# CC834/Heterogeneous-OpenCL-Image-Processing-Engine

Measured on AMD Instinct MI355X. Metric: images_per_sec, higher is better.
Workload: dtype u8

## Files before the change

### heterogeneous-opencl-image-processing-engine_amd/__init__.py

```python
from __future__ import annotations

import ctypes as C
import os
import re
import subprocess

PKG_DIR = os.path.dirname(os.path.abspath(__file__))
ROOT = os.path.dirname(PKG_DIR)
CSRC = os.path.join(PKG_DIR, "csrc")
APPS = os.path.join(PKG_DIR, "apps")
LIB_PATH = os.path.join(PKG_DIR, "libmi_blur.so")
HEADER = os.path.join(ROOT, "include", "mi_blur.h")
HIPCC = os.environ.get("HIPCC", "/opt/rocm/bin/hipcc")
os.environ.setdefault("HIP_FORCE_DEV_KERNARG", "0")
ARCH = "gfx950"

DEVICE_CPU = -1
VARIANT_AUTO, VARIANT_GENERIC, VARIANT_TILED, VARIANT_STREAM, VARIANT_DIRECT = 0, 1, 2, 3, 4
OK, ERR_INVALID, ERR_NO_DEVICE, ERR_NOMEM, ERR_STATE, ERR_UNSUPPORTED = 0, -1, -2, -3, -4, -5
UNIQUE_ID_BYTES = 128
SEP_MAX_RADIUS = 16
MEDIAN_MAX_RADIUS = 7
MORPH_MAX_RADIUS = 16
MORPH_ERODE, MORPH_DILATE, MORPH_GRADIENT = 0, 1, 2
# ... 319 lines not shown
        "mi_blur_warp_perspective_quad": (i, [C.POINTER(C.c_double), C.POINTER(C.c_double), C.POINTER(C.c_double)]),
        "mi_blur_warp_perspective_set_matrix": (i, [C.POINTER(WarpPerspective), C.POINTER(C.c_double), i]),
        "mi_blur_enqueue_warp_perspective": (i, [u8p, u8p, i, i, i, i, C.POINTER(WarpPerspective), vp]),
        "mi_blur_cpu_run_warp_perspective": (i, [u8p, u8p, i, i, i, i, C.POINTER(WarpPerspective), i]),
        "mi_blur_ctx_set_warp_perspective": (i, [vp, C.POINTER(WarpPerspective)]),
        "mi_blur_conv_preset": (i, [i, C.POINTER(Conv)]),
        "mi_blur_enqueue_conv": (i, [u8p, u8p, i, i, i, i, C.POINTER(Conv), vp]),
        "mi_blur_enqueue_conv_band": (i, [u8p, u8p, i, i, i, i, i, C.POINTER(Conv), vp]),
        "mi_blur_cpu_run_conv": (i, [u8p, u8p, i, i, i, i, C.POINTER(Conv), i]),
        "mi_blur_ctx_set_conv": (i, [vp, C.POINTER(Conv)]),
        "mi_blur_fill_synthetic": (None, [u8p, i, i, i, i, i, i]),
        "mi_blur_fnv1a64": (C.c_uint64, [u8p, C.c_size_t]),
        "mi_blur_debug_zc_trace": (i, [vp, C.POINTER(C.c_uint64), i, C.POINTER(i), C.POINTER(C.c_uint)]),
        "mi_blur_debug_xcd_times": (i, [C.POINTER(C.c_uint64), C.POINTER(C.c_uint64), i]),
        "mi_blur_debug_xcd_raw": (i, [C.POINTER(C.c_uint64), C.c_size_t, C.c_size_t]),
        "mi_blur_a1_partition": (None, [i, i, C.c_float, C.POINTER(i), C.POINTER(i)]),
        "mi_blur_shard_range": (None, [C.c_longlong, i, i, C.POINTER(C.c_longlong), C.POINTER(C.c_longlong)]),
        "mi_blur_a2_split": (None, [i, C.c_float, i, C.POINTER(A2Geometry)]),
        "mi_blur_band_of": (None, [i, i, i, i, C.POINTER(Band)]),
        "mi_blur_comm_unique_id": (i, [vp]),
        "mi_blur_comm_init_rank": (i, [C.POINTER(vp), i, i, vp]),
        "mi_blur_comm_init_all": (i, [C.POINTER(vp), i, C.POINTER(i)]),
        "mi_blur_comm_init_p2p": (i, [C.POINTER(vp), i, C.POINTER(i)]),
        "mi_blur_comm_init_pull": (i, [C.POINTER(vp), i, C.POINTER(i)]),
        "mi_blur_comm_destroy": (None, [vp]),
        "mi_blur_comm_info": (i, [vp, C.POINTER(i), C.POINTER(i), C.POINTER(i)]),
        "mi_blur_halo_exchange": (i, [vp, u8p, i, i, i, i, vp]),
        "mi_blur_peer_export": (i, [vp, vp, C.POINTER(C.c_uint64)]),
        "mi_blur_peer_open": (i, [vp, C.c_uint64, C.POINTER(vp)]),
        "mi_blur_peer_close": (i, [vp, C.c_uint64]),
# ... 471 lines not shown
```

### heterogeneous-opencl-image-processing-engine_amd/csrc/blur_kernels.hip

```cpp
#include "kernel_common.h"

#include <math.h>
#include <stdlib.h>
#include <string.h>
#include <mutex>
#include <algorithm>

namespace mi_blur {

__device__ __forceinline__ u16x2 as_pk(uint32_t x) { return __builtin_bit_cast(u16x2, x); }
__device__ __forceinline__ uint32_t as_u32(u16x2 x) { return __builtin_bit_cast(uint32_t, x); }

constexpr uint32_t EVEN_MASK = 0x00ff00ffu;
__device__ __forceinline__ uint32_t even_of(uint32_t x) { return x & EVEN_MASK; }
__device__ __forceinline__ uint32_t odd_of(uint32_t x) { return __builtin_amdgcn_perm(0u, x, 0x0c030c01u); }
__device__ __forceinline__ uint32_t mad6(uint32_t c, uint32_t t) { return as_u32(as_pk(c) * (unsigned short)6 + as_pk(t)); }

constexpr uint32_t sel_left(int C, int q)
{
    uint32_t s = 0;
    for (int j = 0; j < 4; j++) {
        int p = -4 * q + j;
        int idx = ((p % C) + C) % C;
        s |= (uint32_t)idx << (8 * j);
// ... 309 lines not shown
        }
    }
}

constexpr unsigned XCD_DEBUG_SLOTS = 1u << 20;
__device__ __forceinline__ void xcd_time_mark(unsigned long long *t, unsigned long long t0)
{
    if (threadIdx.x == 0 && blockIdx.x < XCD_DEBUG_SLOTS) {
        unsigned id;
        asm volatile("s_getreg_b32 %0, hwreg(HW_REG_XCC_ID)" : "=s"(id));
        t[2u * blockIdx.x] = ((unsigned long long)__builtin_amdgcn_s_memrealtime() << 4) | (id & 7u);
        t[2u * blockIdx.x + 1] = t0;
    }
}

template <int C, int R, int RPG, bool DMA, bool SHFL = false, bool RAG = false>
__global__ __launch_bounds__(256) void blur_tiled_kernel(const TiledParams p)
{
    const unsigned long long t0 = p.xcd_times ? __builtin_amdgcn_s_memrealtime() : 0ull;
    tiled_tile<C, R, RPG, DMA, SHFL, RAG>(p, xcd_map(blockIdx.x, p.nblocks, p.xcd));
    if (p.xcd_times) xcd_time_mark(p.xcd_times, t0);
}

template <int C, int R, int RPG>
__global__ __launch_bounds__(256) void blur_tiled_loop_kernel(const TiledParams p)
{
    for (unsigned L = blockIdx.x; L < p.nblocks; L += gridDim.x) {
        tiled_tile<C, R, RPG, true, false, false>(p, L);
        __syncthreads();
    }
}

template <int C, int R, int RPG, int X>
__global__ __launch_bounds__(256) void blur_tiled_x_kernel(const TiledParams p)
// ... 434 lines not shown
    }
    wait_vmcnt<0>();
}

struct DirectParams {
    const uint8_t *in;
    uint8_t *out;
    long long in_stride, out_stride;
    long long total;
    int pitch, cpr;
    int H, y0, y1;
    int nbands;
    unsigned nblocks;
    int xcd;
    const uint8_t *top, *bottom;
};

template <int C, int R, int BH, bool PEER = false>
__global__ __launch_bounds__(256) void blur_direct_kernel(const DirectParams p)
{
    constexpr int WIN = 2 * R + 1, NR = BH + 2 * R;
    const int lane = threadIdx.x & 63, wave = threadIdx.x >> 6;
    const unsigned B = xcd_map(blockIdx.x, p.nblocks, p.xcd);
    const long long fl = (long long)(B * 4u + (unsigned)wave) * 62 - 1 + lane;
    const bool inrange = fl >= 0 && fl < p.total;
    const unsigned f = (unsigned)(fl < 0 ? 0 : (fl >= p.total ? p.total - 1 : fl));
    const unsigned col = f % (unsigned)p.cpr, t2 = f / (unsigned)p.cpr;
    const unsigned band = t2 % (unsigned)p.nbands;
    const long long img = (long long)(t2 / (unsigned)p.nbands);
    const bool compute = inrange && lane >= 1 && lane <= 62;
    const int row0 = p.y0 + (int)band * BH;
    const int rows_out = compute ? min(BH, p.y1 - row0) : 0;
    const bool at_start = col == 0, at_end = (int)col == p.cpr - 1;
    const bool any_edge = __builtin_amdgcn_ballot_w64(at_start || at_end) != 0ull;
    const uint8_t *src = p.in + img * p.in_stride + (size_t)col * 16u;
    uint8_t *dst = p.out + img * p.out_stride + (size_t)(row0 - p.y0) * (size_t)p.pitch + (size_t)col * 16u;
// ... 36 lines not shown
                    const uint32_t se = (((hw[(j + 2) % WIN][q] << 1) + hw[(j + 1) % WIN][q]) + hw[j % WIN][q]) << 4;
                    const uint32_t so = (((hw[(j + 2) % WIN][4 + q] << 1) + hw[(j + 1) % WIN][4 + q]) + hw[j % WIN][4 + q]) << 4;
                    o[q] = __builtin_amdgcn_perm(so, se, 0x07030501u);
                } else {
                    const uint32_t se = mad6(hw[(j + 3) % WIN][q], ((hw[(j + 2) % WIN][q] + hw[(j + 4) % WIN][q]) << 2) + (hw[(j + 1) % WIN][q] + hw[j % WIN][q]));
                    const uint32_t so = mad6(hw[(j + 3) % WIN][4 + q], ((hw[(j + 2) % WIN][4 + q] + hw[(j + 4) % WIN][4 + q]) << 2) + (hw[(j + 1) % WIN][4 + q] + hw[j % WIN][4 + q]));
                    o[q] = __builtin_amdgcn_perm(so, se, 0x07030501u);
                }
            }
            if (i < rows_out) {
                u32x4 v; v.x = o[0]; v.y = o[1]; v.z = o[2]; v.w = o[3];
                *reinterpret_cast<u32x4 *>(dst + (size_t)i * (size_t)p.pitch) = v;
            }
        }
    }
}

struct GenericParams {
    const uint8_t *in;
    uint8_t *out;
    long long in_stride, out_stride, total;
    int width, channels, pitch;
    int H, y0;
};

template <int R>
__global__ __launch_bounds__(256) void blur_generic_kernel(const GenericParams p)
{
    constexpr int T1[3] = {1, 2, 1};
    constexpr int T2[5] = {1, 4, 6, 4, 1};
// ... 67 lines not shown
{
    return channels >= 1 && channels <= 4 && (long long)width * channels >= 16;
}

bool tiled_eligible(const void *in, const void *out, int width, int channels)
{
    if (channels < 1 || channels > 4) return false;
    const long long pitch = (long long)width * channels;
    return (pitch % 16 == 0) && ((uintptr_t)in % 16 == 0) && ((uintptr_t)out % 16 == 0);
}

static thread_local const char *g_last_kernel = "";
const char *last_kernel() { return g_last_kernel; }
void set_last_kernel(const char *name) { g_last_kernel = name; }

template <int C, int R>
static int launch_tiled_cr(const LaunchDesc &d, const TiledParams &p, dim3 grid, dim3 block, size_t lds,
                           int rpg, bool dma, bool ragged, bool row_shuffle, int experiment)
{
    if (ragged)
        return dispatch<1, 0>(dma, [&](auto DMA) {
            return dispatch<4, 8>(rpg, [&](auto RPG) { return do_launch(blur_tiled_kernel<C, R, RPG, DMA != 0, false, true>, grid, block, lds, d, p); });
        });
    if (d.max_blocks > 0 && dma && rpg != 16 && grid.x > (unsigned)d.max_blocks)
        return dispatch<4, 8>(rpg, [&](auto RPG) { return do_launch(blur_tiled_loop_kernel<C, R, RPG>, dim3((unsigned)d.max_blocks), block, lds, d, p); });
    if (experiment && dma && C == 3 && rpg != 16)
        return dispatch<4, 8>(rpg, [&](auto RPG) { return do_launch(blur_tiled_x_kernel<C, R, RPG, 1 - rowpass_default<R>>, grid, block, lds, d, p); });
    if (row_shuffle && dma)
        return dispatch<16, 4, 8>(rpg, [&](auto RPG) { return do_launch(blur_tiled_kernel<C, R, RPG, true, true>, grid, block, lds, d, p); });
    return dispatch<16, 4, 8>(rpg, [&](auto RPG) {
        return dispatch<1, 0>(dma, [&](auto DMA) { return do_launch(blur_tiled_kernel<C, R, RPG, DMA != 0>, grid, block, lds, d, p); });
    });
}

template <int C>
static int launch_tiled_wide(const LaunchDesc &d, const TiledParams &p, dim3 grid, dim3 block, size_t lds, int rpg, bool ragged)
{
    return dispatch<1, 0>(ragged, [&](auto RAG) {
        return dispatch<4, 8>(rpg, [&](auto RPG) { return do_launch(blur_tiled_kernel<C, 1, RPG, true, false, RAG != 0>, grid, block, lds, d, p); });
    });
}

static bool wide_channels(int channels, int radius) { return channels >= 5 && channels <= 8 && radius == 1; }

template <int R>
static int launch_tiled_r(const LaunchDesc &d, const TiledParams &p, dim3 grid, dim3 block, size_t lds,
                          int rpg, bool dma, bool ragged, bool row_shuffle, int experiment)
{
    if constexpr (R == 1)
        if (d.channels > 4) return dispatch<5, 6, 7, 8>(d.channels, [&](auto C) { return launch_tiled_wide<C>(d, p, grid, block, lds, rpg, ragged); });
    return dispatch<1, 2, 3, 4>(d.channels, [&](auto C) { return launch_tiled_cr<C, R>(d, p, grid, block, lds, rpg, dma, ragged, row_shuffle, experiment); });
}

template <int R>
// ... 101 lines not shown
            if (fused->gate && tun.fused_overlap > 0 && !ragged) {
                const long long ahead = nblocks * tun.fused_overlap / 1000;
                f.gate = fused->gate; f.gate_seq = fused->seq;
                f.gate_block = (unsigned)std::min<long long>(std::max<long long>(nblocks - ahead, 0), (long long)tgrid.x - 1);
            }
            if (p.xcd_times && tgrid.x <= 65536u) p.xcd_times += 2ull * 65536ull * (fused->seq & 15u);
            return dispatch<1, 2>(R, [&](auto Rc) { return launch_fused_r<Rc>(d, p, f, tgrid, block, lds, rpg, ragged); });
        }
        if (ragged) {
            if (!fused->tail_ctr) return MI_BLUR_ERR_UNSUPPORTED;
            f.tail_ctr = fused->tail_ctr; f.ntail = 0; f.nstatic = (unsigned)nblocks; f.nextra = 0;
            g_last_kernel = "blur_fused_tail_kernel";
        }
        return dispatch<1, 2>(R, [&](auto Rc) { return launch_fused_r<Rc>(d, p, f, grid, block, lds, rpg, ragged); });
    }
    return dispatch<1, 2>(R, [&](auto Rc) {
        return launch_tiled_r<Rc>(d, p, grid, block, lds, rpg, tun.stage_dma != 0, ragged, tun.row_shuffle != 0, tun.experiment);
    });
}

int zc_fill_batch(const LaunchDesc &d, ZcGeometry *geo, ZcBatch *b, unsigned *n_tiles)
{
    if (!geo || !b || !d.in || !d.out || d.n_images <= 0) return MI_BLUR_ERR_INVALID;
    Tunables tun = tunables();
    const bool aligned = tiled_eligible(d.in, d.out, d.width, d.channels) && !(d.in_stride % 16) && !(d.out_stride % 16);
    const long long pitch_b = (long long)d.width * d.channels;
    const bool dense = (!d.in_stride || d.in_stride == pitch_b * d.band_rows) && (!d.out_stride || d.out_stride == pitch_b * (d.y1 - d.y0));
    const bool ragged = !aligned && tun.ragged && ragged_eligible(d.width, d.channels) && dense;
    if (!aligned && !ragged) return MI_BLUR_ERR_UNSUPPORTED;
    tun.debug_copy = 0; tun.debug_xcd_times = 0; tun.xcd_remap = 0;
// ... 90 lines not shown
    return dispatch<1, 2, 3, 4>(d.channels, [&](auto C) {
        return dispatch<1, 2>(d.filter->radius, [&](auto R) { return do_launch(blur_stream_kernel<C, R>, grid, block, lds, d, p); });
    });
}

template <int BH>
static int launch_direct_bh(const LaunchDesc &d, const Tunables &tun)
{
    g_last_kernel = "blur_direct_kernel";
    DirectParams p{};
    fill_band(p, d);
    p.cpr = p.pitch / 16; p.y1 = d.y1;
    const dim3 grid = direct_grid(p, d, BH), block(256);
    if (p.total >= 0x7fffffffLL) return MI_BLUR_ERR_INVALID;
    p.xcd = (tun.xcd_remap && p.nblocks >= 16) ? 1 : 0;
    const bool peer = d.halo_top || d.halo_bottom;
    if constexpr (BH != 8) {
        if (peer) return MI_BLUR_ERR_INVALID;
        return dispatch<1, 2>(d.filter->radius, [&](auto R) { return do_launch(blur_direct_kernel<3, R, BH>, grid, block, 0, d, p); });
    } else {
        if (peer) {
            p.top = d.halo_top; p.bottom = d.halo_bottom;
            g_last_kernel = "blur_direct_kernel (peer halo rows)";
            return dispatch<1, 2, 3, 4>(d.channels, [&](auto C) {
                return dispatch<1, 2>(d.filter->radius, [&](auto R) { return do_launch(blur_direct_kernel<C, R, 8, true>, grid, block, 0, d, p); });
            });
        }
        return dispatch<1, 2, 3, 4>(d.channels, [&](auto C) {
            return dispatch<1, 2>(d.filter->radius, [&](auto R) { return do_launch(blur_direct_kernel<C, R, 8>, grid, block, 0, d, p); });
        });
    }
}

static int launch_direct(const LaunchDesc &d, const Tunables &tun)
{
    return dispatch<4, 16, 12, 8>(d.channels == 3 ? tun.direct_bh : 8, [&](auto BH) { return launch_direct_bh<BH>(d, tun); });
}

static int launch_generic(const LaunchDesc &d)
{
    g_last_kernel = "blur_generic_kernel";
    GenericParams p{};
    fill_band(p, d);
    p.total = p.out_stride * d.n_images;
// ... 67 lines not shown
```

### heterogeneous-opencl-image-processing-engine_amd/csrc/blur_launch.h

```cpp
#pragma once
#include <hip/hip_runtime.h>
#include <stdint.h>

#include "filter.h"

namespace mi_blur {

struct LaunchDesc {
    const Filter *filter;
    const uint8_t *in;
    uint8_t *out;
    int width, band_rows, channels;
    int n_images;
    int y0, y1;
    long long in_stride, out_stride;
    int concurrent;
    int max_blocks;
    int variant;
    const uint8_t *halo_top, *halo_bottom;
    hipStream_t stream;
    hipEvent_t start, stop;
};

int launch(const LaunchDesc &d);
int launch_sep(const LaunchDesc &d);
int launch_median(const LaunchDesc &d);
int launch_morph(const LaunchDesc &d);
int launch_bilateral(const LaunchDesc &d);
int launch_conv(const LaunchDesc &d);
int launch_sep_down(const LaunchDesc &d);
int launch_resize(const LaunchDesc &d);
int launch_warp(const LaunchDesc &d);
int launch_warp_persp(const LaunchDesc &d);
void set_last_kernel(const char *name);

struct Tunables;
// ... 60 lines not shown
    int stage_dma; int rpg; int xcd_remap; int debug_copy; int row_shuffle; int prefer_stream; int stream_bh; int zero_copy; int ragged;
    int fused_release;
    int experiment;
    int xcd_run;
    int zero_copy_streams;
    int zero_copy_blocks;
    int stream_updown;
    int prefer_direct;
    int direct_bh;
    int debug_xcd_times;
    int fused_window;
    int fused_tail;
    int fused_adds_per_word;
    int fused_tail_blocks;
    int fused_overlap;
    int zero_copy_server;
    int zero_copy_server_min_kb;
    int staged_server;
    int zero_copy_workers;
    int zero_copy_idle_us;
    int zero_copy_budget;
    int zero_copy_tickets;
    int resident_place_trials;
    int zero_copy_spin;
    int zero_copy_trace;
    int zero_copy_debug_base;
    int zero_copy_events;
};
enum class KnobKind { FLAG, RANGE, ONE_OF };
struct Knob { const char *key; int Tunables::*field; KnobKind kind; int lo, hi, def; const char *env; };
// ... 7 lines not shown
    {"prefer_stream", &Tunables::prefer_stream, KnobKind::FLAG, 0, 1, 0, nullptr},
    {"zero_copy", &Tunables::zero_copy, KnobKind::FLAG, 0, 1, 1, nullptr},
    {"ragged_tiled", &Tunables::ragged, KnobKind::FLAG, 0, 1, 1, nullptr},
    {"stream_band_rows", &Tunables::stream_bh, KnobKind::RANGE, 0, 4096, 0, nullptr},
    {"fused_release", &Tunables::fused_release, KnobKind::FLAG, 0, 1, 0, nullptr},
    {"experiment", &Tunables::experiment, KnobKind::FLAG, 0, 1, 0, nullptr},
    {"stream_updown", &Tunables::stream_updown, KnobKind::FLAG, 0, 1, 1, nullptr},
    {"zero_copy_streams", &Tunables::zero_copy_streams, KnobKind::RANGE, 1, 8, 4, nullptr},
    {"zero_copy_blocks", &Tunables::zero_copy_blocks, KnobKind::RANGE, 0, 1 << 20, 24, nullptr},
    {"prefer_direct", &Tunables::prefer_direct, KnobKind::RANGE, 0, 2, 1, "MI_BLUR_DIRECT"},
    {"direct_bh", &Tunables::direct_bh, KnobKind::ONE_OF, knob_bits(4, 8, 12, 16), 0, 8, nullptr},
    {"fused_adds_per_word", &Tunables::fused_adds_per_word, KnobKind::RANGE, 4, 4096, 32, nullptr},
    {"fused_tail_blocks", &Tunables::fused_tail_blocks, KnobKind::RANGE, 10, 800, 25, nullptr},
    {"fused_tail", &Tunables::fused_tail, KnobKind::RANGE, 0, 500, 30, "MI_BLUR_FUSED_TAIL"},
    {"fused_overlap", &Tunables::fused_overlap, KnobKind::RANGE, 0, 500, 30, "MI_BLUR_FUSED_OVERLAP"},
    {"fused_window", &Tunables::fused_window, KnobKind::RANGE, 1, 4096, 8, nullptr},
    {"debug_xcd_times", &Tunables::debug_xcd_times, KnobKind::FLAG, 0, 1, 0, nullptr},
    {"zero_copy_events", &Tunables::zero_copy_events, KnobKind::FLAG, 0, 1, 1, nullptr},
    {"zero_copy_server", &Tunables::zero_copy_server, KnobKind::FLAG, 0, 1, 1, nullptr},
    {"staged_server", &Tunables::staged_server, KnobKind::FLAG, 0, 1, 1, "MI_BLUR_STAGED_SERVER"},
    {"zero_copy_server_min_kb", &Tunables::zero_copy_server_min_kb, KnobKind::RANGE, 0, 1 << 20, 1280, nullptr},
    {"zero_copy_trace", &Tunables::zero_copy_trace, KnobKind::FLAG, 0, 1, 0, nullptr},
    {"zero_copy_tickets", &Tunables::zero_copy_tickets, KnobKind::FLAG, 0, 1, 1, nullptr},
    {"zero_copy_spin", &Tunables::zero_copy_spin, KnobKind::FLAG, 0, 1, 0, nullptr},
    {"zero_copy_debug_base", &Tunables::zero_copy_debug_base, KnobKind::RANGE, 0, 1 << 20, 0, nullptr},
    {"resident_place_trials", &Tunables::resident_place_trials, KnobKind::RANGE, 0, 8, 4, "MI_BLUR_PLACE_TRIALS"},
    {"zero_copy_workers", &Tunables::zero_copy_workers, KnobKind::RANGE, 1, 2048, 48, nullptr},
    {"zero_copy_idle_us", &Tunables::zero_copy_idle_us, KnobKind::RANGE, 10, 100000, 300, nullptr},
    {"zero_copy_budget", &Tunables::zero_copy_budget, KnobKind::RANGE, 1, 1 << 20, 256, nullptr},
    {"xcd_run", &Tunables::xcd_run, KnobKind::RANGE, 0, 1 << 20, 0, nullptr},
// ... 19 lines not shown
```

### heterogeneous-opencl-image-processing-engine_amd/csrc/kernel_common.h

```cpp
#pragma once
#include "blur_launch.h"
#include "../../include/mi_blur.h"

#include <hip/hip_ext.h>
#include <limits.h>
#include <stdint.h>
#include <type_traits>

namespace mi_blur {

typedef unsigned short u16x2 __attribute__((ext_vector_type(2)));
typedef unsigned int u32x4 __attribute__((ext_vector_type(4)));
typedef unsigned int u32x2 __attribute__((ext_vector_type(2)));

__device__ __forceinline__ unsigned xcd_contiguous(unsigned L, unsigned n)
{
    const unsigned q = n >> 3, r = n & 7u, x = L & 7u, k = L >> 3;
    return (x < r ? x * (q + 1) : r * (q + 1) + (x - r) * q) + k;
}
__device__ __forceinline__ unsigned xcd_runs(unsigned L, unsigned n, unsigned run)
{
    const unsigned span = 8u * run, full = n - n % span;
    if (L >= full) return L;
    const unsigned x = L & 7u, k = L >> 3, j = k / run, o = k - j * run;
// ... 116 lines not shown
    q.src = in + q.img * in_stride;
    return q;
}

static inline int hip_status(hipError_t e) { return e == hipSuccess ? MI_BLUR_OK : MI_BLUR_ERR_HIP_BASE - (int)e; }

template <typename K, typename... A>
static int do_launch(K kernel, dim3 grid, dim3 block, size_t lds, hipStream_t stream, const A &...args)
{
    hipLaunchKernelGGL(kernel, grid, block, lds, stream, args...);
    return hip_status(hipGetLastError());
}
template <typename K, typename... A>
static int do_launch(K kernel, dim3 grid, dim3 block, size_t lds, const LaunchDesc &d, const A &...args)
{
    if (d.start || d.stop)
        hipExtLaunchKernelGGL(kernel, grid, block, lds, d.stream, d.start, d.stop, 0, args...);
    else
        hipLaunchKernelGGL(kernel, grid, block, lds, d.stream, args...);
    return hip_status(hipGetLastError());
}

template <int... Vs, typename F>
static int dispatch(int v, F &&f)
{
    int status = MI_BLUR_ERR_INVALID;
    (void)(... || (v == Vs && (status = f(std::integral_constant<int, Vs>{}), true)));
    return status;
}

// ... 100 lines not shown
```

### heterogeneous-opencl-image-processing-engine_amd/csrc/mi_blur_api.cpp

```cpp
#include "api_internal.h"
#include "blur_launch.h"
#include "cpu_device.h"

#include <sched.h>
#include <time.h>

#include <algorithm>
#include <chrono>
#include <climits>
#include <cmath>
#include <cstdio>
#include <cstdlib>
#include <cstring>
#include <mutex>
#include <new>
#include <deque>
#include <functional>
#include <condition_variable>
#include <thread>
#include <vector>

using namespace mi_blur;

__attribute__((constructor)) static void mi_blur_runtime_defaults() { setenv("HIP_FORCE_DEV_KERNARG", "0", 0); }
// ... 607 lines not shown
    unsigned fused_tpb = 0, fused_wpb = 0, fused_blocks = 0;
    unsigned fused_k = 8;
    int fused_n = 0, fused_batch = 0;
    unsigned fused_passes = 0;
    hipStream_t fused_poll = nullptr;
    unsigned long long *fused_word = nullptr, *fused_word_dev = nullptr;
    unsigned fused_watch_seq = 0;
    bool fused_watched = false;
    bool fused_watch_busy = false;
    hipStream_t fused_second = nullptr;
    hipEvent_t fused_ev = nullptr;
    unsigned fused_seq = 0;
    bool fused_gated = false;
    bool fused_on_second = false;
    bool fused_second_busy = false;
    ZcServer *zc = nullptr;
    std::vector<float> place_ms;
    int place_kept = 0;
    std::vector<CpuJob *> cpu_jobs;
    CpuWorker *cpu_worker = nullptr;
    bool submitted = false;
    bool is_cpu() const { return device == MI_BLUR_DEVICE_CPU; }
};

static bool is_pinned(const void *p)
{
    hipPointerAttribute_t a;
    if (hipPointerGetAttributes(&a, p) != hipSuccess) { (void)hipGetLastError(); return false; }
    return a.type == hipMemoryTypeHost;
}
// ... 338 lines not shown
            if (z.dev) (void)hipFree(z.dev);
            if (z.trace) (void)hipFree(z.trace);
            if (z.ctl) (void)hipHostFree(z.ctl);
            delete c->zc;
            c->zc = nullptr;
        }
        for (auto &s : c->slots) free_slot(s);
        for (auto &t : c->ev_pool) { (void)hipEventDestroy(t.s); (void)hipEventDestroy(t.e); }
        if (c->zc_ref) (void)hipEventDestroy(c->zc_ref);
        if (c->fused_count) (void)hipFree(c->fused_count);
        if (c->fused_host) (void)hipHostFree(c->fused_host);
        if (c->fused_poll) { (void)hipStreamSynchronize(c->fused_poll); (void)hipStreamDestroy(c->fused_poll); }
        if (c->fused_word) (void)hipHostFree(c->fused_word);
        if (c->fused_second) (void)hipStreamDestroy(c->fused_second);
        if (c->fused_ev) (void)hipEventDestroy(c->fused_ev);
        if (c->pool_in) (void)hipFree(c->pool_in);
        if (c->pool_out) (void)hipFree(c->pool_out);
        (void)hipGetLastError();
    }
    delete c;
}

static int zc_server_submit(mi_blur_ctx *c, Slot &s, const LaunchDesc &d, const Tunables &tun)
{
    if (c->filter.kind != FilterKind::BOX) return MI_BLUR_ERR_UNSUPPORTED;
    if (c->slots.size() > ZC_RING) return MI_BLUR_ERR_UNSUPPORTED;
    if (!c->zc) {
        ZcServer *z = new (std::nothrow) ZcServer;
        if (!z) return MI_BLUR_ERR_NOMEM;
        hipError_t e = hipHostMalloc((void **)&z->ctl, sizeof(ZcHostCtl), hipHostMallocDefault);
// ... 516 lines not shown
    const int chunk = std::max(1, (int)std::min<size_t>((size_t)c->pool_images, ((size_t)256 << 20) / c->image_bytes));
    std::vector<uint8_t> host;
    try { host.resize(c->image_bytes * (size_t)chunk); } catch (...) { return MI_BLUR_ERR_NOMEM; }
    for (int i = 0; i < c->pool_images; i += chunk) {
        const int n = std::min(chunk, c->pool_images - i);
        fill_synthetic(host.data(), c->W, c->H, c->C, first_index + i, n, c->n_threads);
        int rc = mi_blur_resident_upload(c, i, host.data(), n);
        if (rc) return rc;
    }
    return MI_BLUR_OK;
}

extern "C" void *mi_blur_resident_in(mi_blur_ctx *c) { return c ? c->pool_in : nullptr; }
extern "C" void *mi_blur_resident_out(mi_blur_ctx *c) { return c ? c->pool_out : nullptr; }

static int fused_join(mi_blur_ctx *c)
{
    if (!c->fused_second_busy) return MI_BLUR_OK;
    HIP_TRY(hipEventRecord(c->fused_ev, c->fused_second));
    for (auto &s : c->slots) HIP_TRY(hipStreamWaitEvent(s.stream, c->fused_ev, 0));
    c->fused_second_busy = false;
    return MI_BLUR_OK;
}

extern "C" int mi_blur_resident_run(mi_blur_ctx *c, int n_images, int batch, int timed_every)
{
    if (!c || n_images < 0 || batch <= 0) return MI_BLUR_ERR_INVALID;
    if (c->filter.kind != FilterKind::BOX) return MI_BLUR_ERR_UNSUPPORTED;
    if (c->is_cpu() || !c->pool_in) return MI_BLUR_ERR_STATE;
    if (batch > c->pool_images) return MI_BLUR_ERR_INVALID;
    HIP_TRY(hipSetDevice(c->device));
    { int rc = fused_join(c); if (rc) return rc; }
    int launch_idx = 0;
    for (int done = 0; done < n_images; done += batch, launch_idx++) {
        const int b = std::min(batch, n_images - done);
        const bool timed = timed_every > 0 && launch_idx % timed_every == 0;
        if (c->cursor + b > c->pool_images) c->cursor = 0;
        Slot &s = c->slots[c->rr];
        c->rr = (c->rr + 1) % (int)c->slots.size();
        LaunchDesc d = ctx_launch(c, c->pool_in + (size_t)c->cursor * c->image_bytes, c->pool_out + (size_t)c->cursor * c->image_bytes,
                                  c->H, b, 0, c->H);
        d.stream = s.stream;
        d.concurrent = (int)c->slots.size();
        if (timed) {
            if (c->ev_used == c->ev_pool.size()) {
                TimedLaunch t{};
                HIP_TRY(hipEventCreate(&t.s));
                HIP_TRY(hipEventCreate(&t.e));
                c->ev_pool.push_back(t);
            }
            d.start = c->ev_pool[c->ev_used].s; d.stop = c->ev_pool[c->ev_used].e;
            c->ev_used++;
        }
        int rc = launch(d);
        if (rc) return rc;
        c->cursor += b;
        c->tm.launches += 1;
        if (timed) { c->timed_launches += 1; c->timed_bytes_alg += 2ull * c->image_bytes * (uint64_t)b; }
    }
    c->tm.images += (uint64_t)n_images;
    c->tm.bytes_alg += 2ull * c->image_bytes * (uint64_t)n_images;
    return MI_BLUR_OK;
}

static size_t fused_words(int cap) { return 8 * (size_t)cap + 16384; }
constexpr size_t FUSED_TAIL_BANK = 32, FUSED_GATE_WORD = 64, FUSED_EXTRA_WORDS = 96;

extern "C" int mi_blur_resident_run_fused(mi_blur_ctx *c, int n_images, int batch, int timed)
{
    if (!c || n_images <= 0 || batch <= 0) return MI_BLUR_ERR_INVALID;
    if (c->filter.kind != FilterKind::BOX) return MI_BLUR_ERR_UNSUPPORTED;
    if (c->is_cpu() || !c->pool_in) return MI_BLUR_ERR_STATE;
    if (n_images > c->pool_images) return MI_BLUR_ERR_INVALID;
    HIP_TRY(hipSetDevice(c->device));
    const int nb = (n_images + batch - 1) / batch;
    if (nb > c->fused_cap) {
        for (auto &s : c->slots) HIP_TRY(hipStreamSynchronize(s.stream));
        if (c->fused_second) HIP_TRY(hipStreamSynchronize(c->fused_second));
        c->fused_second_busy = false; c->fused_gated = false;
        if (c->fused_count) { (void)hipFree(c->fused_count); c->fused_count = nullptr; }
        if (c->fused_host) { (void)hipHostFree(c->fused_host); c->fused_host = nullptr; }
        c->fused_cap = 0;
        const int cap = std::max(nb, c->pool_images);
        HIP_TRY(hipMalloc((void **)&c->fused_count, sizeof(unsigned) * (fused_words(cap) + FUSED_EXTRA_WORDS)));
        HIP_TRY(hipMemset(c->fused_count + fused_words(cap), 0, sizeof(unsigned) * FUSED_EXTRA_WORDS));
        HIP_TRY(hipMemcpy(c->fused_count + fused_words(cap) + FUSED_GATE_WORD, &c->fused_seq, sizeof(unsigned), hipMemcpyHostToDevice));
        HIP_TRY(hipDeviceSynchronize());
        HIP_TRY(hipHostMalloc((void **)&c->fused_host, sizeof(unsigned) * fused_words(cap), hipHostMallocDefault));
        c->fused_cap = cap;
        c->fused_passes = 0;
    }
    if (!c->fused_poll) {
        HIP_TRY(hipStreamCreateWithFlags(&c->fused_poll, hipStreamNonBlocking));
        HIP_TRY(hipMemcpyAsync(c->fused_host, c->fused_count, sizeof(unsigned) * fused_words(c->fused_cap), hipMemcpyDeviceToHost, c->fused_poll));
        HIP_TRY(hipStreamSynchronize(c->fused_poll));
    }
    if (c->cursor + n_images > c->pool_images) c->cursor = 0;
    Slot &s = c->slots[0];
    LaunchDesc d = ctx_launch(c, c->pool_in + (size_t)c->cursor * c->image_bytes, c->pool_out + (size_t)c->cursor * c->image_bytes,
                              c->H, n_images, 0, c->H);
    d.variant = MI_BLUR_VARIANT_TILED; d.stream = s.stream;
    const Tunables tun = tunables();
    unsigned tpb = 0, wpb = 0, blocks = 0, kcnt = 8, ntail = 0;
    unsigned *const extra = c->fused_count + fused_words(c->fused_cap);
    const unsigned seq = c->fused_seq + 1u;
    FusedDesc f{c->fused_count, batch, &tpb, &wpb, &blocks, &tun, true, extra + (tun.fused_overlap > 0 ? (seq & 1u) * FUSED_TAIL_BANK : 0), (long long)fused_words(c->fused_cap), &kcnt,
                &ntail, nullptr, seq};
    int rc = launch_fused(d, f);
    if (rc) return rc;
    const bool same = n_images == c->fused_n && batch == c->fused_batch && tpb == c->fused_tpb && wpb == c->fused_wpb && kcnt == c->fused_k &&
                      blocks == c->fused_blocks && c->fused_passes > 0 && c->fused_passes < (1u << 20);
    const bool raises = tun.fused_overlap > 0 && ntail > 0 && !(timed & 2) && tiled_eligible(d.in, d.out, c->W, c->C);
    const bool overlap = raises && same && c->fused_gated;
    if (overlap) {
        d.stream = c->fused_on_second ? s.stream : c->fused_second;
        rc = launch_fused_gate(extra + FUSED_GATE_WORD, c->fused_seq, d.stream);
        if (rc) return rc;
    } else {
        rc = fused_join(c);
        if (rc) return rc;
    }
    if (raises) f.gate = extra + FUSED_GATE_WORD;
    if (same) {
        c->fused_passes += 1;
    } else {
        if (c->fused_watch_busy) { HIP_TRY(hipStreamSynchronize(c->fused_second)); c->fused_watch_busy = false; }
        HIP_TRY(hipMemsetAsync(c->fused_count, 0, sizeof(unsigned) * (size_t)kcnt * (size_t)nb, s.stream));
        c->fused_n = n_images; c->fused_batch = batch; c->fused_passes = 1;
        c->fused_tpb = tpb; c->fused_wpb = wpb; c->fused_blocks = blocks; c->fused_k = kcnt;
    }
    c->fused_batches = nb;
    c->fused_watched = false;
    if (timed & 2) {
        if (c->fused_passes == 1) HIP_TRY(hipStreamSynchronize(s.stream));
        if (!c->fused_word) {
            HIP_TRY(hipHostMalloc((void **)&c->fused_word, sizeof(unsigned long long), hipHostMallocDefault));
            *c->fused_word = 0;
// ... 2 lines not shown
    }
    if (timed & 1) {
        if (c->ev_used == c->ev_pool.size()) {
            TimedLaunch t{};
            HIP_TRY(hipEventCreate(&t.s));
            HIP_TRY(hipEventCreate(&t.e));
            c->ev_pool.push_back(t);
        }
        d.start = c->ev_pool[c->ev_used].s; d.stop = c->ev_pool[c->ev_used].e;
        c->ev_used++;
    }
    f.geometry_only = false;
    rc = launch_fused(d, f);
    if (rc) { c->fused_passes = 0; c->fused_batches = 0; c->fused_gated = false; return rc; }
    c->fused_seq = seq;
    c->fused_gated = raises;
    c->fused_on_second = d.stream == c->fused_second;
    if (c->fused_on_second) c->fused_second_busy = true;
    c->cursor += n_images;
    c->tm.launches += 1;
    c->tm.images += (uint64_t)n_images;
    c->tm.bytes_alg += 2ull * c->image_bytes * (uint64_t)n_images;
    if (timed & 1) { c->timed_launches += 1; c->timed_bytes_alg += 2ull * c->image_bytes * (uint64_t)n_images; }
    if (timed & 2) {
        c->fused_watch_seq += 1;
        rc = launch_fused_watch(c->fused_count, (unsigned)nb, tpb, blocks, wpb * c->fused_passes, c->fused_word_dev, c->fused_watch_seq, c->fused_second, c->fused_k);
        if (rc) return rc;
        c->fused_watched = true;
        c->fused_watch_busy = true;
        c->fused_second_busy = true;
    }
// ... 110 lines not shown

extern "C" int mi_blur_cpu_run_conv(const uint8_t *in, uint8_t *out, int width, int height, int channels, int n_images,
                                    const mi_blur_conv *k, int n_threads)
{
    Filter f;
    return cpu_run_filter(filter_conv(k, &f), f, in, out, width, height, channels, n_images, n_threads);
}

extern "C" void mi_blur_fill_synthetic(uint8_t *host, int width, int height, int channels, int first_index,
                                       int n_images, int n_threads)
{
    if (host && width > 0 && height > 0 && channels > 0)
        fill_synthetic(host, width, height, channels, first_index, n_images, n_threads);
}

extern "C" int mi_blur_debug_xcd_times(uint64_t end_ticks[8], uint64_t begin_ticks[8], int rearm)
{
    unsigned long long *d = debug_xcd_buffer();
    if (!d) return MI_BLUR_ERR_NOMEM;
    const size_t n = debug_xcd_slots();
    std::vector<unsigned long long> h;
    try { h.resize(2 * n); } catch (...) { return MI_BLUR_ERR_NOMEM; }
    HIP_TRY(hipDeviceSynchronize());
    HIP_TRY(hipMemcpy(h.data(), d, 16 * n, hipMemcpyDeviceToHost));
    uint64_t e[8] = {0, 0, 0, 0, 0, 0, 0, 0}, b[8];
    for (int i = 0; i < 8; i++) b[i] = ~0ull;
    for (size_t i = 0; i < n; i++) {
        if (!h[2 * i]) continue;
        const int x = (int)(h[2 * i] & 7u);
        e[x] = std::max<uint64_t>(e[x], h[2 * i] >> 4);
// ... 77 lines not shown
```

### include/mi_blur.h

```cpp
#ifndef MI_BLUR_H
#define MI_BLUR_H

#include <stddef.h>
#include <stdint.h>

#ifdef __cplusplus
extern "C" {
#endif

#define MI_BLUR_VERSION 1
#define MI_BLUR_DEVICE_CPU (-1)

typedef enum mi_blur_status {
    MI_BLUR_OK = 0,
    MI_BLUR_ERR_INVALID = -1,
    MI_BLUR_ERR_NO_DEVICE = -2,
    MI_BLUR_ERR_NOMEM = -3,
    MI_BLUR_ERR_STATE = -4,
    MI_BLUR_ERR_UNSUPPORTED = -5,
    MI_BLUR_ERR_HIP_BASE = -1000,
    MI_BLUR_ERR_RCCL_BASE = -2000
} mi_blur_status;

typedef enum mi_blur_variant {
// ... 228 lines not shown
} mi_blur_conv_preset_id;
int mi_blur_conv_preset(int preset, mi_blur_conv *k);

int mi_blur_enqueue_conv(const uint8_t *d_in, uint8_t *d_out, int width, int height, int channels, int n_images,
                         const mi_blur_conv *k, void *stream);
int mi_blur_enqueue_conv_band(const uint8_t *d_in, uint8_t *d_out, int width, int band_rows, int channels,
                              int out_row_begin, int out_row_end, const mi_blur_conv *k, void *stream);
int mi_blur_cpu_run_conv(const uint8_t *in, uint8_t *out, int width, int height, int channels, int n_images,
                         const mi_blur_conv *k, int n_threads);
int mi_blur_ctx_set_conv(mi_blur_ctx *ctx, const mi_blur_conv *k);

int mi_blur_debug_xcd_times(uint64_t end_ticks[8], uint64_t begin_ticks[8], int rearm);

int mi_blur_debug_xcd_raw(uint64_t *out, size_t first_slot, size_t n_slots);

int mi_blur_debug_zc_trace(mi_blur_ctx *ctx, uint64_t *out, int max_batches, int *n_workers, unsigned *batches_published);

void mi_blur_fill_synthetic(uint8_t *host, int width, int height, int channels,
                            int first_index, int n_images, int n_threads);
uint64_t mi_blur_fnv1a64(const uint8_t *host, size_t n);

void mi_blur_a1_partition(int mode, int batch_count, float gpu_ratio, int *n_cpu, int *n_gpu);
void mi_blur_shard_range(long long n_units, int g, int G, long long *begin, long long *end);

typedef struct mi_blur_a2_geometry {
    int split_row;
    int cpu_input_rows, cpu_output_rows;
    int gpu_input_rows, gpu_output_rows;
} mi_blur_a2_geometry;
void mi_blur_a2_split(int height, float gpu_ratio, int halo, mi_blur_a2_geometry *g);
// ... 38 lines not shown
```

Before: 15.46 million.

## Overlap consecutive plain resident launches via device gate word on second stream

Plain resident runs can now overlap back-to-back kernel launches. A chosen block near the tail of each tiled/direct kernel raises a device gate word, and the next launch goes on an alternate stream behind a gate-wait kernel. This lets the next batch start while the previous kernel's tail drains. In exchange it adds a geometry-only dry-run launch per batch, a gate kernel launch, and cross-stream ordering complexity, which risks races if the two kernels touch the same buffers.

```diff
diff --git a/heterogeneous-opencl-image-processing-engine_amd/__init__.py b/heterogeneous-opencl-image-processing-engine_amd/__init__.py
--- a/heterogeneous-opencl-image-processing-engine_amd/__init__.py
+++ b/heterogeneous-opencl-image-processing-engine_amd/__init__.py
@@ -357,6 +357,7 @@
         "mi_blur_debug_zc_trace": (i, [vp, C.POINTER(C.c_uint64), i, C.POINTER(i), C.POINTER(C.c_uint)]),
         "mi_blur_debug_xcd_times": (i, [C.POINTER(C.c_uint64), C.POINTER(C.c_uint64), i]),
         "mi_blur_debug_xcd_raw": (i, [C.POINTER(C.c_uint64), C.c_size_t, C.c_size_t]),
+        "mi_blur_debug_gated_launches": (C.c_uint64, [vp]),
         "mi_blur_a1_partition": (None, [i, i, C.c_float, C.POINTER(i), C.POINTER(i)]),
         "mi_blur_shard_range": (None, [C.c_longlong, i, i, C.POINTER(C.c_longlong), C.POINTER(C.c_longlong)]),
         "mi_blur_a2_split": (None, [i, C.c_float, i, C.POINTER(A2Geometry)]),
diff --git a/heterogeneous-opencl-image-processing-engine_amd/csrc/blur_kernels.hip b/heterogeneous-opencl-image-processing-engine_amd/csrc/blur_kernels.hip
--- a/heterogeneous-opencl-image-processing-engine_amd/csrc/blur_kernels.hip
+++ b/heterogeneous-opencl-image-processing-engine_amd/csrc/blur_kernels.hip
@@ -347,10 +347,20 @@
     }
 }
 
+struct GateArg {
+    unsigned *gate;
+    unsigned gate_block, gate_seq;
+};
+__device__ __forceinline__ void raise_gate(const GateArg &g)
+{
+    if (g.gate && blockIdx.x == g.gate_block && threadIdx.x == 0) __hip_atomic_store(g.gate, g.gate_seq, __ATOMIC_RELAXED, __HIP_MEMORY_SCOPE_AGENT);
+}
+
 template <int C, int R, int RPG, bool DMA, bool SHFL = false, bool RAG = false>
-__global__ __launch_bounds__(256) void blur_tiled_kernel(const TiledParams p)
+__global__ __launch_bounds__(256) void blur_tiled_kernel(const TiledParams p, const GateArg g)
 {
     const unsigned long long t0 = p.xcd_times ? __builtin_amdgcn_s_memrealtime() : 0ull;
+    if (__builtin_expect(g.gate != nullptr, 0)) raise_gate(g);
     tiled_tile<C, R, RPG, DMA, SHFL, RAG>(p, xcd_map(blockIdx.x, p.nblocks, p.xcd));
     if (p.xcd_times) xcd_time_mark(p.xcd_times, t0);
 }
@@ -815,12 +825,15 @@
     unsigned nblocks;
     int xcd;
     const uint8_t *top, *bottom;
+    unsigned long long *xcd_times;
 };
 
 template <int C, int R, int BH, bool PEER = false>
-__global__ __launch_bounds__(256) void blur_direct_kernel(const DirectParams p)
+__global__ __launch_bounds__(256) void blur_direct_kernel(const DirectParams p, const GateArg g)
 {
     constexpr int WIN = 2 * R + 1, NR = BH + 2 * R;
+    const unsigned long long t0 = p.xcd_times ? __builtin_amdgcn_s_memrealtime() : 0ull;
+    raise_gate(g);
     const int lane = threadIdx.x & 63, wave = threadIdx.x >> 6;
     const unsigned B = xcd_map(blockIdx.x, p.nblocks, p.xcd);
     const long long fl = (long long)(B * 4u + (unsigned)wave) * 62 - 1 + lane;
@@ -887,6 +900,7 @@
             }
         }
     }
+    if (p.xcd_times) xcd_time_mark(p.xcd_times, t0);
 }
 
 struct GenericParams {
@@ -984,22 +998,42 @@
 const char *last_kernel() { return g_last_kernel; }
 void set_last_kernel(const char *name) { g_last_kernel = name; }
 
+static GateArg gate_arg(const LaunchDesc &d, unsigned nblocks)
+{
+    GateArg g{};
+    if (!d.gate) return g;
+    d.gate->blocks = nblocks;
+    if (d.gate->word && !d.gate->geometry_only && nblocks > 0) {
+        const long long ahead = (long long)nblocks * d.gate->per_mille / 1000;
+        g.gate = d.gate->word; g.gate_seq = d.gate->seq;
+        g.gate_block = (unsigned)std::min<long long>(std::max<long long>((long long)nblocks - ahead, 0), (long long)nblocks - 1);
+    }
+    return g;
+}
+static unsigned long long *debug_xcd_region(const Tunables &tun, const LaunchDesc &d, unsigned nblocks)
+{
+    if (!tun.debug_xcd_times) return nullptr;
+    unsigned long long *t = debug_xcd_buffer();
+    return t && nblocks <= 65536u ? t + 2ull * 65536ull * (d.debug_region & 15u) : t;
+}
+
 template <int C, int R>
 static int launch_tiled_cr(const LaunchDesc &d, const TiledParams &p, dim3 grid, dim3 block, size_t lds,
                            int rpg, bool dma, bool ragged, bool row_shuffle, int experiment)
 {
     if (ragged)
         return dispatch<1, 0>(dma, [&](auto DMA) {
-            return dispatch<4, 8>(rpg, [&](auto RPG) { return do_launch(blur_tiled_kernel<C, R, RPG, DMA != 0, false, true>, grid, block, lds, d, p); });
+            return dispatch<4, 8>(rpg, [&](auto RPG) { return do_launch(blur_tiled_kernel<C, R, RPG, DMA != 0, false, true>, grid, block, lds, d, p, GateArg{}); });
         });
     if (d.max_blocks > 0 && dma && rpg != 16 && grid.x > (unsigned)d.max_blocks)
         return dispatch<4, 8>(rpg, [&](auto RPG) { return do_launch(blur_tiled_loop_kernel<C, R, RPG>, dim3((unsigned)d.max_blocks), block, lds, d, p); });
     if (experiment && dma && C == 3 && rpg != 16)
         return dispatch<4, 8>(rpg, [&](auto RPG) { return do_launch(blur_tiled_x_kernel<C, R, RPG, 1 - rowpass_default<R>>, grid, block, lds, d, p); });
     if (row_shuffle && dma)
-        return dispatch<16, 4, 8>(rpg, [&](auto RPG) { return do_launch(blur_tiled_kernel<C, R, RPG, true, true>, grid, block, lds, d, p); });
+        return dispatch<16, 4, 8>(rpg, [&](auto RPG) { return do_launch(blur_tiled_kernel<C, R, RPG, true, true>, grid, block, lds, d, p, GateArg{}); });
+    const GateArg g = dma ? gate_arg(d, grid.x) : GateArg{};
     return dispatch<16, 4, 8>(rpg, [&](auto RPG) {
-        return dispatch<1, 0>(dma, [&](auto DMA) { return do_launch(blur_tiled_kernel<C, R, RPG, DMA != 0>, grid, block, lds, d, p); });
+        return dispatch<1, 0>(dma, [&](auto DMA) { return do_launch(blur_tiled_kernel<C, R, RPG, DMA != 0>, grid, block, lds, d, p, g); });
     });
 }
 
@@ -1007,7 +1041,7 @@
 static int launch_tiled_wide(const LaunchDesc &d, const TiledParams &p, dim3 grid, dim3 block, size_t lds, int rpg, bool ragged)
 {
     return dispatch<1, 0>(ragged, [&](auto RAG) {
-        return dispatch<4, 8>(rpg, [&](auto RPG) { return do_launch(blur_tiled_kernel<C, 1, RPG, true, false, RAG != 0>, grid, block, lds, d, p); });
+        return dispatch<4, 8>(rpg, [&](auto RPG) { return do_launch(blur_tiled_kernel<C, 1, RPG, true, false, RAG != 0>, grid, block, lds, d, p, GateArg{}); });
     });
 }
 
@@ -1139,6 +1173,7 @@
         }
         return dispatch<1, 2>(R, [&](auto Rc) { return launch_fused_r<Rc>(d, p, f, grid, block, lds, rpg, ragged); });
     }
+    p.xcd_times = debug_xcd_region(tun, d, p.nblocks);
     return dispatch<1, 2>(R, [&](auto Rc) {
         return launch_tiled_r<Rc>(d, p, grid, block, lds, rpg, tun.stage_dma != 0, ragged, tun.row_shuffle != 0, tun.experiment);
     });
@@ -1259,20 +1294,22 @@
     const dim3 grid = direct_grid(p, d, BH), block(256);
     if (p.total >= 0x7fffffffLL) return MI_BLUR_ERR_INVALID;
     p.xcd = (tun.xcd_remap && p.nblocks >= 16) ? 1 : 0;
+    p.xcd_times = debug_xcd_region(tun, d, p.nblocks);
     const bool peer = d.halo_top || d.halo_bottom;
     if constexpr (BH != 8) {
         if (peer) return MI_BLUR_ERR_INVALID;
-        return dispatch<1, 2>(d.filter->radius, [&](auto R) { return do_launch(blur_direct_kernel<3, R, BH>, grid, block, 0, d, p); });
+        return dispatch<1, 2>(d.filter->radius, [&](auto R) { return do_launch(blur_direct_kernel<3, R, BH>, grid, block, 0, d, p, gate_arg(d, grid.x)); });
     } else {
         if (peer) {
             p.top = d.halo_top; p.bottom = d.halo_bottom;
             g_last_kernel = "blur_direct_kernel (peer halo rows)";
             return dispatch<1, 2, 3, 4>(d.channels, [&](auto C) {
-                return dispatch<1, 2>(d.filter->radius, [&](auto R) { return do_launch(blur_direct_kernel<C, R, 8, true>, grid, block, 0, d, p); });
+                return dispatch<1, 2>(d.filter->radius, [&](auto R) { return do_launch(blur_direct_kernel<C, R, 8, true>, grid, block, 0, d, p, GateArg{}); });
             });
         }
+        const GateArg g = gate_arg(d, grid.x);
         return dispatch<1, 2, 3, 4>(d.channels, [&](auto C) {
-            return dispatch<1, 2>(d.filter->radius, [&](auto R) { return do_launch(blur_direct_kernel<C, R, 8>, grid, block, 0, d, p); });
+            return dispatch<1, 2>(d.filter->radius, [&](auto R) { return do_launch(blur_direct_kernel<C, R, 8>, grid, block, 0, d, p, g); });
         });
     }
 }
diff --git a/heterogeneous-opencl-image-processing-engine_amd/csrc/blur_launch.h b/heterogeneous-opencl-image-processing-engine_amd/csrc/blur_launch.h
--- a/heterogeneous-opencl-image-processing-engine_amd/csrc/blur_launch.h
+++ b/heterogeneous-opencl-image-processing-engine_amd/csrc/blur_launch.h
@@ -5,6 +5,14 @@
 #include "filter.h"
 
 namespace mi_blur {
+
+struct PlainGate {
+    unsigned *word;
+    unsigned seq;
+    int per_mille;
+    bool geometry_only;
+    long long blocks;
+};
 
 struct LaunchDesc {
     const Filter *filter;
@@ -20,6 +28,8 @@
     const uint8_t *halo_top, *halo_bottom;
     hipStream_t stream;
     hipEvent_t start, stop;
+    PlainGate *gate;
+    unsigned debug_region;
 };
 
 int launch(const LaunchDesc &d);
@@ -110,6 +120,8 @@
     int fused_adds_per_word;
     int fused_tail_blocks;
     int fused_overlap;
+    int plain_overlap;
+    int plain_overlap_min_blocks;
     int zero_copy_server;
     int zero_copy_server_min_kb;
     int staged_server;
@@ -147,6 +159,8 @@
     {"fused_tail_blocks", &Tunables::fused_tail_blocks, KnobKind::RANGE, 10, 800, 25, nullptr},
     {"fused_tail", &Tunables::fused_tail, KnobKind::RANGE, 0, 500, 30, "MI_BLUR_FUSED_TAIL"},
     {"fused_overlap", &Tunables::fused_overlap, KnobKind::RANGE, 0, 500, 30, "MI_BLUR_FUSED_OVERLAP"},
+    {"plain_overlap", &Tunables::plain_overlap, KnobKind::RANGE, 0, 500, 30, "MI_BLUR_PLAIN_OVERLAP"},
+    {"plain_overlap_min_blocks", &Tunables::plain_overlap_min_blocks, KnobKind::RANGE, 1, 1 << 30, 8192, nullptr},
     {"fused_window", &Tunables::fused_window, KnobKind::RANGE, 1, 4096, 8, nullptr},
     {"debug_xcd_times", &Tunables::debug_xcd_times, KnobKind::FLAG, 0, 1, 0, nullptr},
     {"zero_copy_events", &Tunables::zero_copy_events, KnobKind::FLAG, 0, 1, 1, nullptr},
diff --git a/heterogeneous-opencl-image-processing-engine_amd/csrc/kernel_common.h b/heterogeneous-opencl-image-processing-engine_amd/csrc/kernel_common.h
--- a/heterogeneous-opencl-image-processing-engine_amd/csrc/kernel_common.h
+++ b/heterogeneous-opencl-image-processing-engine_amd/csrc/kernel_common.h
@@ -154,6 +154,7 @@
 template <typename K, typename... A>
 static int do_launch(K kernel, dim3 grid, dim3 block, size_t lds, const LaunchDesc &d, const A &...args)
 {
+    if (d.gate && d.gate->geometry_only) return MI_BLUR_OK;
     if (d.start || d.stop)
         hipExtLaunchKernelGGL(kernel, grid, block, lds, d.stream, d.start, d.stop, 0, args...);
     else
diff --git a/heterogeneous-opencl-image-processing-engine_amd/csrc/mi_blur_api.cpp b/heterogeneous-opencl-image-processing-engine_amd/csrc/mi_blur_api.cpp
--- a/heterogeneous-opencl-image-processing-engine_amd/csrc/mi_blur_api.cpp
+++ b/heterogeneous-opencl-image-processing-engine_amd/csrc/mi_blur_api.cpp
@@ -645,6 +645,10 @@
     bool fused_gated = false;
     bool fused_on_second = false;
     bool fused_second_busy = false;
+    unsigned *gate_word = nullptr;
+    bool gate_plain = false;
+    uint64_t gated_launches = 0;
+    unsigned plain_launches = 0;
     ZcServer *zc = nullptr;
     std::vector<float> place_ms;
     int place_kept = 0;
@@ -1013,6 +1017,7 @@
         if (c->fused_word) (void)hipHostFree(c->fused_word);
         if (c->fused_second) (void)hipStreamDestroy(c->fused_second);
         if (c->fused_ev) (void)hipEventDestroy(c->fused_ev);
+        if (c->gate_word) (void)hipFree(c->gate_word);
         if (c->pool_in) (void)hipFree(c->pool_in);
         if (c->pool_out) (void)hipFree(c->pool_out);
         (void)hipGetLastError();
@@ -1559,6 +1564,19 @@
 extern "C" void *mi_blur_resident_in(mi_blur_ctx *c) { return c ? c->pool_in : nullptr; }
 extern "C" void *mi_blur_resident_out(mi_blur_ctx *c) { return c ? c->pool_out : nullptr; }
 
+static int make_gate_word(mi_blur_ctx *c)
+{
+    if (c->gate_word) return MI_BLUR_OK;
+    unsigned *w = nullptr;
+    HIP_TRY(hipMalloc((void **)&w, 128));
+    if (hipMemcpy(w, &c->fused_seq, sizeof(unsigned), hipMemcpyHostToDevice) != hipSuccess || hipDeviceSynchronize() != hipSuccess) {
+        (void)hipGetLastError(); (void)hipFree(w);
+        return MI_BLUR_ERR_STATE;
+    }
+    c->gate_word = w;
+    return MI_BLUR_OK;
+}
+
 static int fused_join(mi_blur_ctx *c)
 {
     if (!c->fused_second_busy) return MI_BLUR_OK;
@@ -1575,7 +1593,9 @@
     if (c->is_cpu() || !c->pool_in) return MI_BLUR_ERR_STATE;
     if (batch > c->pool_images) return MI_BLUR_ERR_INVALID;
     HIP_TRY(hipSetDevice(c->device));
-    { int rc = fused_join(c); if (rc) return rc; }
+    const Tunables tun = tunables();
+    const bool may_overlap = c->slots.size() == 1 && tun.plain_overlap > 0 && ((long long)c->W * c->C) % 16 == 0;
+    if (may_overlap) { int rc = make_gate_word(c); if (rc) return rc; }
     int launch_idx = 0;
     for (int done = 0; done < n_images; done += batch, launch_idx++) {
         const int b = std::min(batch, n_images - done);
@@ -1587,6 +1607,29 @@
                                   c->H, b, 0, c->H);
         d.stream = s.stream;
         d.concurrent = (int)c->slots.size();
+        d.debug_region = c->plain_launches++;
+        PlainGate pg{};
+        bool raises = false;
+        if (may_overlap) {
+            pg.geometry_only = true; d.gate = &pg;
+            int rc = launch(d);
+            if (rc) return rc;
+            raises = pg.blocks >= (long long)tun.plain_overlap_min_blocks;
+            d.gate = nullptr;
+        }
+        if (raises && c->fused_gated && c->gate_plain) {
+            d.stream = c->fused_on_second ? s.stream : c->fused_second;
+            int rc = launch_fused_gate(c->gate_word, c->fused_seq, d.stream);
+            if (rc) return rc;
+            c->gated_launches += 1;
+        } else {
+            int rc = fused_join(c);
+            if (rc) return rc;
+        }
+        if (raises) {
+            pg = PlainGate{c->gate_word, c->fused_seq + 1u, tun.plain_overlap, false, 0};
+            d.gate = &pg;
+        }
         if (timed) {
             if (c->ev_used == c->ev_pool.size()) {
                 TimedLaunch t{};
@@ -1599,6 +1642,15 @@
         }
         int rc = launch(d);
         if (rc) return rc;
+        if (raises && pg.blocks > 0) {
+            c->fused_seq += 1u;
+            c->fused_gated = true; c->gate_plain = true;
+            c->fused_on_second = d.stream == c->fused_second;
+            if (c->fused_on_second) c->fused_second_busy = true;
+        } else {
+            c->fused_gated = false;
+            if (d.stream == c->fused_second) c->fused_second_busy = true;
+        }
         c->cursor += b;
         c->tm.launches += 1;
         if (timed) { c->timed_launches += 1; c->timed_bytes_alg += 2ull * c->image_bytes * (uint64_t)b; }
@@ -1609,7 +1661,7 @@
 }
 
 static size_t fused_words(int cap) { return 8 * (size_t)cap + 16384; }
-constexpr size_t FUSED_TAIL_BANK = 32, FUSED_GATE_WORD = 64, FUSED_EXTRA_WORDS = 96;
+constexpr size_t FUSED_TAIL_BANK = 32, FUSED_EXTRA_WORDS = 64;
 
 extern "C" int mi_blur_resident_run_fused(mi_blur_ctx *c, int n_images, int batch, int timed)
 {
@@ -1629,12 +1681,12 @@
         const int cap = std::max(nb, c->pool_images);
         HIP_TRY(hipMalloc((void **)&c->fused_count, sizeof(unsigned) * (fused_words(cap) + FUSED_EXTRA_WORDS)));
         HIP_TRY(hipMemset(c->fused_count + fused_words(cap), 0, sizeof(unsigned) * FUSED_EXTRA_WORDS));
-        HIP_TRY(hipMemcpy(c->fused_count + fused_words(cap) + FUSED_GATE_WORD, &c->fused_seq, sizeof(unsigned), hipMemcpyHostToDevice));
         HIP_TRY(hipDeviceSynchronize());
         HIP_TRY(hipHostMalloc((void **)&c->fused_host, sizeof(unsigned) * fused_words(cap), hipHostMallocDefault));
         c->fused_cap = cap;
         c->fused_passes = 0;
     }
+    { int rc = make_gate_word(c); if (rc) return rc; }
     if (!c->fused_poll) {
         HIP_TRY(hipStreamCreateWithFlags(&c->fused_poll, hipStreamNonBlocking));
         HIP_TRY(hipMemcpyAsync(c->fused_host, c->fused_count, sizeof(unsigned) * fused_words(c->fused_cap), hipMemcpyDeviceToHost, c->fused_poll));
@@ -1656,16 +1708,16 @@
     const bool same = n_images == c->fused_n && batch == c->fused_batch && tpb == c->fused_tpb && wpb == c->fused_wpb && kcnt == c->fused_k &&
                       blocks == c->fused_blocks && c->fused_passes > 0 && c->fused_passes < (1u << 20);
     const bool raises = tun.fused_overlap > 0 && ntail > 0 && !(timed & 2) && tiled_eligible(d.in, d.out, c->W, c->C);
-    const bool overlap = raises && same && c->fused_gated;
+    const bool overlap = raises && same && c->fused_gated && !c->gate_plain;
     if (overlap) {
         d.stream = c->fused_on_second ? s.stream : c->fused_second;
-        rc = launch_fused_gate(extra + FUSED_GATE_WORD, c->fused_seq, d.stream);
+        rc = launch_fused_gate(c->gate_word, c->fused_seq, d.stream);
         if (rc) return rc;
     } else {
         rc = fused_join(c);
         if (rc) return rc;
     }
-    if (raises) f.gate = extra + FUSED_GATE_WORD;
+    if (raises) f.gate = c->gate_word;
     if (same) {
         c->fused_passes += 1;
     } else {
@@ -1698,7 +1750,7 @@
     rc = launch_fused(d, f);
     if (rc) { c->fused_passes = 0; c->fused_batches = 0; c->fused_gated = false; return rc; }
     c->fused_seq = seq;
-    c->fused_gated = raises;
+    c->fused_gated = raises; c->gate_plain = false;
     c->fused_on_second = d.stream == c->fused_second;
     if (c->fused_on_second) c->fused_second_busy = true;
     c->cursor += n_images;
@@ -1839,6 +1891,8 @@
         fill_synthetic(host, width, height, channels, first_index, n_images, n_threads);
 }
 
+extern "C" uint64_t mi_blur_debug_gated_launches(mi_blur_ctx *c) { return c ? c->gated_launches : 0; }
+
 extern "C" int mi_blur_debug_xcd_times(uint64_t end_ticks[8], uint64_t begin_ticks[8], int rearm)
 {
     unsigned long long *d = debug_xcd_buffer();
diff --git a/include/mi_blur.h b/include/mi_blur.h
--- a/include/mi_blur.h
+++ b/include/mi_blur.h
@@ -266,6 +266,8 @@
 
 int mi_blur_debug_xcd_raw(uint64_t *out, size_t first_slot, size_t n_slots);
 
+uint64_t mi_blur_debug_gated_launches(mi_blur_ctx *ctx);
+
 int mi_blur_debug_zc_trace(mi_blur_ctx *ctx, uint64_t *out, int max_batches, int *n_workers, unsigned *batches_published);
 
 void mi_blur_fill_synthetic(uint8_t *host, int width, int height, int channels,
```

Measured after the change: 15.31 million. About the same (-1.0%).
